# redwarp/kmeans-gpu

Hardware: AMD Instinct MI355X
Metric: pixels/sec per Lloyd iteration (8192x8192, k=256) (higher is better)
Workload: dtype f32; 1 GPU; synthetic uniform RGBA 8192x8192 (seed 0x5EED0003), k=256, one Lloyd iteration = update + assign (labels written every iteration) + accumulate; width=8192, height=8192, k=256, collective_backend=none (one rank), collective_ranks=1, label_pass=before the next iteration, update=by the last launch of the assign pass (kmg_lloyd_assign_update)

## Files before the change

### kmeans-gpu_amd/csrc/kmg_cube.hip

```cpp

#include "kmg_internal.h"
#include "kmg_table_dev.h"

#include <hip/hip_fp16.h>
#include <stdlib.h>

namespace kmg {

typedef float f32x2 __attribute__((ext_vector_type(2)));


namespace {

constexpr uint32_t kMaxListed = 32;
constexpr uint32_t kMaxLong = 256;
constexpr uint32_t kLongFlag = 0x200u;

__device__ __forceinline__ uint32_t sel3(uint32_t i, uint32_t x0, uint32_t x1, uint32_t x2)
{
    return i == 0u ? x0 : (i == 1u ? x1 : x2);
}

__device__ __forceinline__ int round_dir(int g, int m)
{
// ... 8 lines not shown
{
    v |= dpp_u32<kDppXor1>(v);
    v |= dpp_u32<kDppXor2>(v);
    v |= dpp_u32<kDppHalfMirror>(v);
    return v;
}

__device__ __forceinline__ uint32_t group8_min_u32(uint32_t v)
{
    v = min(v, dpp_u32<kDppXor1>(v));
    v = min(v, dpp_u32<kDppXor2>(v));
    v = min(v, dpp_u32<kDppHalfMirror>(v));
    return v;
}

__device__ __forceinline__ uint32_t group8_max_u32(uint32_t v)
{
    v = max(v, dpp_u32<kDppXor1>(v));
    v = max(v, dpp_u32<kDppXor2>(v));
    v = max(v, dpp_u32<kDppHalfMirror>(v));
    return v;
}



__device__ __forceinline__ uint32_t cell_pair_entry(const uint32_t idx[8], uint32_t occ, uint32_t lane)
{
    uint32_t rem = occ;
    uint32_t lab0 = 0, lab1 = 0, lab2 = 0, cnt0 = 0, cnt1 = 0, cnt2 = 0, msk0 = 0, msk1 = 0, msk2 = 0, n_occ = 0;
#pragma unroll
    for (int t = 0; t < 3; ++t) {
        const unsigned long long any = __ballot(rem != 0u);
        if (any) {
            uint32_t mine = 0;
#pragma unroll
            for (int q = 7; q >= 0; --q) mine = ((rem >> q) & 1u) ? idx[q] : mine;
            const uint32_t v = lane_value(mine, (uint32_t)__builtin_ctzll(any));
            uint32_t mm = 0;
#pragma unroll
            for (int q = 0; q < 8; ++q) mm |= (idx[q] == v ? 1u : 0u) << q;
            mm &= rem;
            rem &= ~mm;
            const uint32_t packed = wave_add_u32((uint32_t)__builtin_popcount(mm) | (t == 0 ? (uint32_t)__builtin_popcount(occ) << 10 : 0u));
            const uint32_t c = packed & 1023u;
            if (t == 0) { lab0 = v; msk0 = mm; cnt0 = c; n_occ = packed >> 10; }
            if (t == 1) { lab1 = v; msk1 = mm; cnt1 = c; }
            if (t == 2) { lab2 = v; msk2 = mm; cnt2 = c; }
// ... 17 lines not shown
    const int gx = (int)((hR & 1023u) * nA) - (int)((hA & 1023u) * nR);
    const int gy = (int)(((hR >> 10) & 1023u) * nA) - (int)(((hA >> 10) & 1023u) * nR);
    const int gz = (int)((hR >> 20) * nA) - (int)((hA >> 20) * nR);
    const int ax = gx < 0 ? -gx : gx, ay = gy < 0 ? -gy : gy, az = gz < 0 ? -gz : gz;
    const int m = ax > ay ? (ax > az ? ax : az) : (ay > az ? ay : az);
    int nx = 2, ny = 0, nz = 0;
    if (m > 0) { nx = round_dir(gx, m); ny = round_dir(gy, m); nz = round_dir(gz, m); }

    const int xl = (int)(((lane >> 5) & 1u) * 4u + ((lane >> 1) & 3u));
    const int yl = (int)(((lane >> 4) & 1u) * 4u + (lane & 1u) * 2u);
    const int zl = (int)(((lane >> 3) & 1u) * 4u);
    const int bias = 7 * ((nx < 0 ? -nx : 0) + (ny < 0 ? -ny : 0) + (nz < 0 ? -nz : 0));
    const int p0 = nx * xl + ny * yl + nz * zl + bias;
    int p[8];
#pragma unroll
    for (int q = 0; q < 8; ++q) p[q] = p0 + ny * (q >> 2) + nz * (q & 3);
    const uint32_t notB = occ & ~mB;
    uint32_t tl = 63u, hi = 64u;
#pragma unroll
    for (int q = 0; q < 8; ++q) {
        if ((rest >> q) & 1u) tl = min(tl, (uint32_t)p[q]);
        if ((notB >> q) & 1u) hi = min(hi, (uint32_t)(63 - p[q]));
    }
    u16x2 packed = __builtin_bit_cast(u16x2, tl | (hi << 16));
    packed = __builtin_elementwise_min(packed, __builtin_bit_cast(u16x2, dpp_u32<kDppXor1>(__builtin_bit_cast(uint32_t, packed))));
    packed = __builtin_elementwise_min(packed, __builtin_bit_cast(u16x2, dpp_u32<kDppXor2>(__builtin_bit_cast(uint32_t, packed))));
    packed = __builtin_elementwise_min(packed, __builtin_bit_cast(u16x2, dpp_u32<kDppHalfMirror>(__builtin_bit_cast(uint32_t, packed))));
    packed = __builtin_elementwise_min(packed, __builtin_bit_cast(u16x2, dpp_u32<kDppMirror>(__builtin_bit_cast(uint32_t, packed))));
    packed = __builtin_elementwise_min(packed, __builtin_bit_cast(u16x2, (uint32_t)__builtin_amdgcn_update_dpp(-1, (int)__builtin_bit_cast(uint32_t, packed), 0x142, 0xA, 0xF, false)));
    packed = __builtin_elementwise_min(packed, __builtin_bit_cast(u16x2, (uint32_t)__builtin_amdgcn_update_dpp(-1, (int)__builtin_bit_cast(uint32_t, packed), 0x143, 0xC, 0xF, false)));
    const uint32_t pk = lane_value(__builtin_bit_cast(uint32_t, packed), 63);
    const int tlo = (int)(pk & 0xFFFFu);
    const int thi = 63 - (int)(pk >> 16);
    const int w = thi + 1 > tlo ? thi + 1 - tlo : 0;
    const uint32_t code = pair_dir_code(nx, ny, nz);
    if (w <= 6) return pair_entry(labA, labB, code, (uint32_t)tlo, (uint32_t)w);
    uint32_t low = 0, high = 0;
#pragma unroll
    for (int q = 0; q < 8; ++q) {
        if ((occ >> q) & 1u) { low += p[q] < tlo ? 1u : 0u; high += p[q] > thi ? 1u : 0u; }
    }
    const uint32_t lh = wave_add_u32(low | (high << 10));
    if ((lh & 1023u) >= (lh >> 10)) return pair_entry(labA, labB, code, (uint32_t)tlo, 7u);
    const int range = 7 * ((nx < 0 ? -nx : nx) + (ny < 0 ? -ny : ny) + (nz < 0 ? -nz : nz));
    return pair_entry(labB, labA, pair_dir_code(-nx, -ny, -nz), (uint32_t)(range - thi), 7u);
}

__device__ __forceinline__ uint32_t merge_state(uint32_t a, uint32_t b)
{
    return (a == kSubEmpty) ? b : ((b == kSubEmpty || b == a) ? a : (uint32_t)kSubMixed);
}

template <typename LabelT>
__device__ __forceinline__ void store_labels64(LabelT *dst64, uint32_t label, uint32_t lane)
{
    if (sizeof(LabelT) == 1) {
        const uint32_t t = label | (dpp_u32<kDppXor1>(label) << 8);
        const uint32_t u = t | (dpp_u32<kDppXor2>(t) << 16);
        if ((lane & 3u) == 0u) reinterpret_cast<uint32_t *>(dst64)[lane >> 2] = u;
    } else {
        const uint32_t t = label | (dpp_u32<kDppXor1>(label) << 16);
        if ((lane & 1u) == 0u) reinterpret_cast<uint32_t *>(dst64)[lane >> 1] = t;
    }
}


struct alignas(16) CellWork {
    uint16_t list[kMaxListed];
    unsigned long long br[4];
    uint32_t npop;
    uint32_t scan_set;
    uint32_t pad[6];
};
static_assert(sizeof(CellWork) == 128, "CellWork layout");

constexpr uint32_t kPairPending = 0xFFFFFFFEu;

constexpr uint32_t kLongSegs = 16, kLongSegCap = kCells / kLongSegs, kLongCount = 0, kLongCells = 64;
constexpr size_t kListsWords = kLongCells + kCells;
constexpr uint32_t kItemCands = 12;

__device__ __forceinline__ void flush_bins(const unsigned long long *bins, uint32_t k, uint32_t repl, uint32_t bin_stride,
                                           int64_t *sums, uint32_t n_rows)
{
    __syncthreads();
    unsigned long long *row = reinterpret_cast<unsigned long long *>(sums) + (uint64_t)(blockIdx.x % n_rows) * 4ull * k;
    for (uint32_t i = threadIdx.x; i < 4u * k; i += blockDim.x) {
        unsigned long long v = 0ull;
        for (uint32_t r = 0; r < repl; ++r) v += bins[(uint64_t)r * bin_stride + i];
        if (v) atomicAdd(row + i, v);
    }
}

__device__ __forceinline__ uint2 long_list_stage(const float4 *s_cent, const unsigned long long *s_masks, uint16_t *s_long,
                                              unsigned long long *s_sub, float4 sb0, float4 sb1, float4 sb2, uint32_t npop,
                                              uint32_t words, uint64_t *sub_masks_cell)
{
    const uint32_t lane = threadIdx.x & 63u;
    const uint32_t sub_of_lane = lane >> 3, cand_of_lane = lane & 7u;
// ... 1263 lines not shown
        KMG_STAMP(0);
        uint32_t task = wv < waves_used ? blockIdx.x * waves_used + wv : tasks;
        if (bal_state) task = min(s_bal[64u + wv], tasks);
        const uint32_t prime = tasks % 2053u ? 2053u : 1031u;
        const uint32_t pos = (uint32_t)(((uint64_t)task * prime) % tasks) + ci * tasks;
        const bool valid = task < tasks && ci < cpw && pos < n_work;
        const uint32_t cell = valid ? ((SUMS && n_work != kCells) ? work[1u + pos] : pos) : 0u;
        const uint32_t sc = cell * 8u + sub;
        const uint32_t cell_a = (uint32_t)__builtin_amdgcn_ds_bpermute((int)(((lane >> 4) * 8u) << 2), (int)cell);
        const uint32_t cell_b = (uint32_t)__builtin_amdgcn_ds_bpermute((int)(((4u + (lane >> 4)) * 8u) << 2), (int)cell);
        const float cbv_a = reinterpret_cast<const float *>(bounds + cell_a)[lane & 15u];
        const float cbv_b = reinterpret_cast<const float *>(bounds + cell_b)[lane & 15u];
        const float4 *sbp = reinterpret_cast<const float4 *>(sub_bounds + sc);
        const float4 sb0 = sbp[0], sb1 = sbp[1], sb2 = sbp[2];
        longlong2 g01 = {0, 0}, g23 = {0, 1};
        long long cell_sum = 0;
        if (SUMS) {
            const longlong2 *sp = reinterpret_cast<const longlong2 *>(sub_agg + (uint64_t)sc * 4u);
            g01 = sp[0]; g23 = sp[1];
            cell_sum = agg[4ull * cell + (sub & 3u)];
        }
        uint2 occ8 = make_uint2(0xFFFFFFFFu, 0xFFFFFFFFu);
        if (occ_bits) occ8 = *reinterpret_cast<const uint2 *>(occ_bits + (uint64_t)cell * 64u + sub * 8u);
        if (sub == 0u) s_cell[slot] = cell;

        float *s_cb = reinterpret_cast<float *>(s_lbl + (size_t)wv * 8u * kCellColours);
        s_cb[lane] = cbv_a;
        s_cb[64u + lane] = cbv_b;
        __builtin_amdgcn_wave_barrier();
        for (uint32_t c = 0; c < cpw; ++c) {
            const uint32_t ccell = lane_value(cell, c * 8u);
            const bool cvalid = lane_value((uint32_t)valid, c * 8u) != 0u;
            const float4 *cq = reinterpret_cast<const float4 *>(s_cb + c * 16u);
            const float4 q0 = cq[0], q1 = cq[1], q2 = cq[2];
            CellBounds cb;
            cb.L0 = q0.x; cb.L1 = q0.y; cb.a0 = q0.z; cb.a1 = q0.w;
            cb.b0 = q1.x; cb.b1 = q1.y; cb.C0 = q1.z; cb.C1 = q1.w;
            cb.wC0 = q2.x; cb.wC1 = q2.y; cb.wH0 = q2.z; cb.wH1 = q2.w;
            float lo[4], U = 3.0e38f;
#pragma unroll
            for (int w = 0; w < 4; ++w) {
                const KeyRange r = key_range(cb, c4[w].x, c4[w].y, c4[w].z, c4[w].w);
                lo[w] = r.lo;
                U = fminf(U, r.hi);
            }
            const float Us = mask_threshold(wave_min(U));
// ... 31 lines not shown
        if (listed) {
            CellBounds sb;
            sb.L0 = sb0.x; sb.L1 = sb0.y; sb.a0 = sb0.z; sb.a1 = sb0.w;
            sb.b0 = sb1.x; sb.b1 = sb1.y; sb.C0 = sb1.z; sb.C1 = sb1.w;
            sb.wC0 = sb2.x; sb.wC1 = sb2.y; sb.wH0 = sb2.z; sb.wH1 = sb2.w;
            uint32_t Ubest = 0x7F7FFFE0u;
            for (uint32_t p = 0; p < npop; ++p) {
                const float4 c = s_cent[s_list[slot * kMaxListed + p]];
                Ubest = min(Ubest, ((float_to_bits(key_range(sb, c.x, c.y, c.z, c.w).hi) + 31u) & ~31u) | p);
            }
            const float Us = mask_threshold(bits_to_float(Ubest & ~31u));
            for (uint32_t p = 0; p < npop; ++p) {
                const float4 c = s_cent[s_list[slot * kMaxListed + p]];
                sm |= (key_range(sb, c.x, c.y, c.z, c.w).lo <= Us ? 1u : 0u) << p;
            }
            istar = Ubest & 31u;
            ubits = Ubest & ~31u;
        }
        const uint32_t np0 = (uint32_t)__builtin_popcount(sm);
        const bool was_decided = listed && occupied && np0 == 1u;
        const bool mine = listed && occupied && np0 > 1u;
        s_mask[threadIdx.x] = sm;
        *reinterpret_cast<uint2 *>(s_occ + slot * 64u + sub * 8u) = occ8;
        const uint32_t others = (mine && dominance) ? sm & ~(1u << istar) : 0u;
        if (others) {
            s_ref[threadIdx.x] = ubits | istar;
            const uint32_t nt = (uint32_t)__builtin_popcount(others);
            uint32_t at = atomicAdd(&s_count[8u + wv], nt);
            for (uint32_t m = others; m && at < kOneTests; m &= m - 1u, ++at)
                s_test[wv * kOneTests + at] = (uint16_t)((lane << 5) | (uint32_t)__builtin_ctz(m));
        }
        KMG_STAMP(2);
        __builtin_amdgcn_fence(__ATOMIC_RELEASE, "workgroup");
        __builtin_amdgcn_wave_barrier();
        __builtin_amdgcn_fence(__ATOMIC_ACQUIRE, "workgroup");
        if (dominance) {
            const uint32_t n_tests = min(__builtin_amdgcn_readfirstlane(s_count[8u + wv]), kOneTests);
            for (uint32_t t = lane; t < n_tests; t += 64u) {
                const uint32_t ent = (uint32_t)s_test[wv * kOneTests + t];
                const uint32_t e = wv * 64u + (ent >> 5), tp = ent & 31u;
                const uint32_t r = s_ref[e];
                const float4 cj = s_cent[s_list[(e >> 3) * kMaxListed + tp]], ci4 = s_cent[s_list[(e >> 3) * kMaxListed + (r & 31u)]];
                HalfModel mdl;
                mdl.load(sub_affine, (uint64_t)s_cell[e >> 3] * 8u + (e & 7u));
                if (dominated(mdl, cj, ci4, bits_to_float(r & ~31u))) atomicAnd(&s_mask[e], ~(1u << tp));
            }
// ... 66 lines not shown
                    for (uint32_t m = un; m; m &= m - 1u, ++q) {
                        const uint32_t cc = (uint32_t)s_list[slot * kMaxListed + (uint32_t)__builtin_ctz(m)] << (8u * (q & 3u));
                        iw0 |= q < 4u ? cc : 0u; iw1 |= (q >= 4u && q < 8u) ? cc : 0u; iw2 |= q >= 8u ? cc : 0u;
                    }
                }
                s_item[i_base + bits_below_lane(item_b)] = make_uint4(slot | (sub << 7) | (s1 << 10) | (n_un << 14) | (type << 30), iw0, iw1, iw2);
            }
            if (stats) {
                st_single += (uint32_t)__builtin_popcountll(__ballot(single && sub == 0u));
                st_multi += (uint32_t)__builtin_popcountll(__ballot(valid && !single && sub == 0u));
                st_unlisted += (uint32_t)__builtin_popcountll(__ballot(unlisted && sub == 0u));
                st_decided += (uint32_t)__builtin_popcountll(__ballot(was_decided));
                st_scanned += (uint32_t)__builtin_popcountll(__ballot(mine || (unlisted && occupied)));
                st_cands += wave_add_u32(mine ? np0 : ((unlisted && occupied) ? npop : 0u));
                st_removed += wave_add_u32((uint32_t)__builtin_popcount(sm & ~nm));
                st_one += (uint32_t)__builtin_popcountll(__ballot(one));
            }
        }
        KMG_STAMP(4);
        __syncthreads();
        const uint32_t n_items = s_count[0];
        KMG_STAMP_VALUE(8, n_items); KMG_STAMP_VALUE(10, s_count[8]);

        auto cell_entry = [&](const uint32_t ps) {
            const uint32_t pcell = __builtin_amdgcn_readfirstlane(s_cell[ps]);
            const uint2 lv = *reinterpret_cast<const uint2 *>(s_lbl + ps * kCellColours + lane * 8u);
            uint32_t e = kPairPending;
            if (!(flags & kCubeNoEntries)) {
                const uint32_t occ = (uint32_t)s_occ[ps * 64u + lane];
                uint32_t idx[8];
#pragma unroll
                for (uint32_t q = 0; q < 4u; ++q) { idx[q] = (lv.x >> (8u * q)) & 0xFFu; idx[4u + q] = (lv.y >> (8u * q)) & 0xFFu; }
                e = cell_pair_entry(idx, occ, lane);
            }
            if (lane == 0u) pair_entries[pcell] = e;
            *reinterpret_cast<uint2 *>(colour_labels + (uint64_t)pcell * kCellColours + lane * 8u) = lv;
        };

        {
            uint32_t A_h = 0u, A_w0 = 0u, A_w1 = 0u, A_w2 = 0u, B_h = 0u, B_w0 = 0u, B_w1 = 0u, B_w2 = 0u, C_h = 0u, C_w0 = 0u, C_w1 = 0u, C_w2 = 0u;
            float4 A_v0, A_v1, B_v0, B_v1, C_v0, C_v1;
            uint32_t A_c0 = 1u, A_c1 = 1u, B_c0 = 1u, B_c1 = 1u, C_c0 = 1u, C_c1 = 1u;
            long long A_g = 0, B_g = 0, C_g = 0;
            bool A_ok = false, B_ok = false, C_ok = false;
#define KMG_REQUEST_ITEM(X)                                                                                       \
            do {                                                                                                  \
                uint32_t next_ = 0u;                                                                              \
                if (lane == 0u) next_ = atomicAdd(&s_count[4], 1u);                                               \
                next_ = __builtin_amdgcn_readfirstlane(next_);                                                    \
                X##_ok = next_ < n_items;                                                                         \
                const uint4 it_ = s_item[next_ < n_items ? next_ : 0u];                                           \
                X##_h = __builtin_amdgcn_readfirstlane(it_.x); X##_w0 = __builtin_amdgcn_readfirstlane(it_.y);    \
                X##_w1 = __builtin_amdgcn_readfirstlane(it_.z); X##_w2 = __builtin_amdgcn_readfirstlane(it_.w);   \
                const uint32_t cell_ = __builtin_amdgcn_readfirstlane(s_cell[X##_h & 127u]);                       \
                const uint32_t c0_ = cell_ * kCellColours + ((X##_h >> 7) & 7u) * 64u + lane;                     \
                const uint32_t c1_ = cell_ * kCellColours + ((X##_h >> 10) & 7u) * 64u + lane;    \
// ... 165 lines not shown
}
#define env_grid(name, dflt) grid_or(KMG_TOOLS_ENV(name), (dflt))

uint32_t cube_replicas(uint32_t k)
{
    uint32_t r = 4;
    if (const char *e = KMG_TOOLS_ENV("KMG_CUBE_REPL")) { const int v = atoi(e); if (v == 1 || v == 2 || v == 4 || v == 8) r = (uint32_t)v; }
    while (r > 1u && (uint64_t)r * (k * 32ull + 32ull) > 33024ull) r >>= 1;
    return r;
}

size_t cube_work_bytes() { return sizeof(CellWork) * (size_t)kCells + sizeof(uint32_t) * kListsWords; }

bool cube_single_launch(uint32_t k, uint32_t flags)
{
    return k <= kSmallMaxK || (k <= 256u && !(flags & kCubeHot));
}

hipError_t launch_cube(const CubePass &c, hipStream_t st)
{
    const uint32_t k = c.k;
    uint32_t n_rows = c.n_rows, flags = c.flags;
    const CubeBalance *balance = c.balance;
    const CubeTail tl = (c.tail && c.hist && n_rows <= 1u) ? *c.tail : CubeTail();
    const uint32_t kpad = (k + 63u) & ~63u;
    const bool with_sums = c.hist != nullptr;
    const uint32_t repl = with_sums ? cube_replicas(k) : 1u;
    const size_t lds_stage = sizeof(float4) * kpad + (with_sums ? sizeof(unsigned long long) * 4ull * k : 0) +
                             sizeof(uint32_t) * (kBlock / 64) * kMaxListed + sizeof(unsigned long long) * (kBlock / 64) * (kpad / 64u) +
                             (k <= 256 ? (kBlock / 64) * (32u * sizeof(unsigned long long) + kMaxLong * sizeof(uint16_t)) : 0u);
    const size_t lds_scan = sizeof(float4) * kpad + (with_sums ? sizeof(unsigned long long) * (4ull * k + 4ull) * repl : 0) +
                            sizeof(float4) * (kScanBlock / 64) * kMaxListed + (k <= 256 ? 1u : 2u) * (kScanBlock / 64) * kCellColours;
    {
        const size_t lds_max = device_info().lds_max;
        if (lds_stage > lds_max || lds_scan > lds_max) return hipErrorInvalidValue;
    }
    const size_t lds_max_dev = device_info().lds_max;
    static const bool small_on = tools_env_int(KMG_TOOLS_ENV("KMG_CUBE_SMALL"), 1) != 0;
    if (k <= kSmallMaxK && small_on) {
        static const uint32_t g_small = env_grid("KMG_SMALL_GRID", kCells / kSmallCells);
        const uint32_t kp = k <= 8u ? 8u : (k <= 16u ? 16u : 32u);
        const size_t lds = sizeof(float4) * kp + (with_sums ? sizeof(unsigned long long) * (4ull * k + 4ull) * kSmallRepl : 0) +
                           (size_t)kSmallCells * kCellColours + sizeof(uint32_t) * kSmallBlock * 2u + sizeof(uint32_t) * kSmallCells +
                           sizeof(uint32_t) * 4u + sizeof(uint16_t) * (kSmallBlock + kSmallCells + kSmallTests) + kSmallBlock;
        if (!n_rows) n_rows = 1u;
        static const bool split = tools_env_int(KMG_TOOLS_ENV("KMG_CUBE_SMALL"), 1) == 2;
// ... 88 lines not shown
```

### kmeans-gpu_amd/csrc/kmg_lloyd.hip

```cpp

#include <math.h>

#include "kmg_state.h"

static void drop_events(kmg_lloyd *s)
{
    for (ProfEvent &e : s->events) { s->pool.push_back(e.e0); s->pool.push_back(e.e1); }
    s->events.clear();
}

static void destroy_events(kmg_lloyd *s)
{
    drop_events(s);
    for (hipEvent_t e : s->pool) (void)hipEventDestroy(e);
    s->pool.clear();
}

static int side_flush(kmg_lloyd *s, hipStream_t st)
{
    for (int i = 0; i < 2; ++i)
        if (s->lab_pending[i]) {
            HIP_TRY(hipStreamWaitEvent(st, s->ev_lab[i], 0));
            s->lab_pending[i] = false;
        }
// ... 30 lines not shown
{
    if (t.balance_work != work) { t.balance_work = work; t.balance_pass = 0; }
    CubeBalance b;
    b.state = t.d_balance;
    b.pass = t.balance_pass++;
    return b;
}

static hipError_t cube_pass(kmg_lloyd *s, hipStream_t st, int64_t *d_sums, uint32_t rows, bool share, bool balance, uint32_t flags = 0u,
                            const CubeTail *tail = nullptr, unsigned long long *d_stage = nullptr)
{
    ColourTable &t = s->tab;
    const uint32_t *work = share ? share_or_work(t) : t.d_work;
    CubeBalance bal;
    if (balance) bal = next_balance(t, work);
    CubePass c;
    c.hist = t.d_hist; c.agg = t.d_agg; c.sub_agg = t.d_sub_agg; c.occ_bits = t.d_occ; c.work = work;
    c.bounds = s->p->d_bounds; c.sub_bounds = s->p->d_sub_bounds; c.lab_table = s->p->d_lab_table;
    c.cent = s->d_cent; c.k = s->k;
    c.masks = t.d_masks; c.cell_work = t.d_cell_work; c.colour_labels = t.d_colour_labels; c.sub_table = t.d_sub;
    c.sums = d_sums; c.n_rows = rows; c.flags = flags | hot_flag(t); c.stats = d_stage; c.tail = tail;
    c.sub_affine = affine_for(s->p, s->k, st);
    c.balance = balance ? &bal : nullptr;
    return launch_cube(c, st);
}

static int label_pass(kmg_lloyd *s, const uint8_t *d_rgba, uint64_t n, uint32_t *d_labels, hipStream_t st, const CubeTail *tail = nullptr,
                      int64_t *acc = nullptr)
{
    const ColourTable &t = s->tab;
    PROF_LAUNCH(s, KMG_K_LABELS, st, launch_labels((const uint32_t *)d_rgba, n, t.d_colour_labels, t.d_sub, s->k, nullptr, d_labels, st,
                                                   s->reserve_cus, hot_list(t), tail, acc));
    return KMG_OK;
}

static CubeTail make_tail(const kmg_lloyd *s, int64_t *acc_out, bool do_update)
{
    return CubeTail{acc_out, do_update ? 1 : 0, s->p->opt.convergence, s->d_cent, s->d_nconv};
}

static int check_unweighted(const kmg_lloyd *s, const char *call)
{
    if (s->weighted)
        return fail(KMG_ERR_INVALID_ARGUMENT, "%s: the object's sums are weighted (kmg_lloyd_set_weighting): the colour table counts pixels", call);
    return KMG_OK;
}

// ... 108 lines not shown
    if (e == hipSuccess) e = launch_sub_affine(p->d_lab_table, p->d_sub_bounds, a, st);
    if (e == hipSuccess) e = hipStreamSynchronize(st);
    if (e != hipSuccess) {
        (void)hipGetLastError();
        if (a) (void)hipFree(a);
        p->affine_failed = true;
        return nullptr;
    }
    p->d_sub_affine = a;
    return a;
}

static int tables_from_histogram(kmg_lloyd *s, uint64_t n_pixels, hipStream_t st)
{
    ColourTable &t = s->tab;
    HIP_TRY(launch_cell_aggregates(t.d_hist, s->p->d_lab_table, t.d_agg, t.d_sub_agg, t.d_occ, st));
    HIP_TRY(launch_work_list(t.d_agg, t.d_work, s->k <= 256 ? n_pixels : 0, st));
    HIP_TRY(hipMemcpyAsync(&t.n_hot, t.d_work + kCells + 1, sizeof(uint32_t), hipMemcpyDeviceToHost, st));
    HIP_TRY(hipMemcpyAsync(&t.n_occ, t.d_work, sizeof(uint32_t), hipMemcpyDeviceToHost, st));
    HIP_TRY(hipStreamSynchronize(st));
    if (const char *e = KMG_TOOLS_ENV("KMG_HOT_CELLS")) { if (e[0] == '0') t.n_hot = 0; }
    t.d_work_share = nullptr;
    t.balance_work = nullptr;
    return KMG_OK;
}

static int bind_image_impl(kmg_lloyd *s, const uint8_t *d_rgba, uint64_t n, void *stream, bool want_tie, uint64_t first_index)
{
    if (!s || !d_rgba || n == 0) return fail(KMG_ERR_INVALID_ARGUMENT, "bad bind_image arguments");
    if (s->side) HIP_TRY(hipStreamSynchronize(s->side));
    s->lab_pending[0] = s->lab_pending[1] = false;
    KMG_TRY(check_pixel_count(n));
    HIP_TRY(hipSetDevice(s->p->device));
    KMG_TRY(ensure_bounds(s->p, S(stream)));
    ColourTable &t = s->tab;
    if (!t.d_hist) {
        const size_t sizes[11] = {sizeof(uint32_t) << 24, sizeof(int64_t) * 4ull * kCells, sizeof(int64_t) * 4ull * kSubCells,
                                  (size_t)1 << 21, cube_work_bytes(), cube_masks_bytes(s->k),
                                  sizeof(uint32_t) * kWorkWords, (size_t)(s->k <= 256 ? 1 : 2) << 24, sub_table_bytes(),
                                  sizeof(uint32_t) * (kCells + 1), cube_balance_bytes()};
        size_t need = 0;
        for (size_t b : sizes) need += pad256(b);
        const hipError_t e = block_take(s->p, need, &t.blk, &t.blk_cap);
        if (e != hipSuccess) {
            t.blk = nullptr; t.blk_cap = 0;
            return fail_hip(e, "colour table allocation");
        }
        size_t off = 0;
        t.d_hist = (uint32_t *)carve(t.blk, off, sizes[0]);
        t.d_agg = (int64_t *)carve(t.blk, off, sizes[1]);
        t.d_sub_agg = (int64_t *)carve(t.blk, off, sizes[2]);
        t.d_occ = (uint8_t *)carve(t.blk, off, sizes[3]);
        t.d_cell_work = carve(t.blk, off, sizes[4]);
        t.d_masks = (uint64_t *)carve(t.blk, off, sizes[5]);
        t.d_work = (uint32_t *)carve(t.blk, off, sizes[6]);
        t.d_colour_labels = carve(t.blk, off, sizes[7]);
        t.d_sub = (uint16_t *)carve(t.blk, off, sizes[8]);
        t.share_buf = (uint32_t *)carve(t.blk, off, sizes[9]);
        t.d_balance = (uint16_t *)carve(t.blk, off, sizes[10]);
    }
    t.d_work_share = nullptr;
    t.balance_work = nullptr;
    t.rgba = nullptr;
    t.tables_valid = false;
    t.tie_valid = false;
    t.bound_by_init = false;
    t.bound_by_caller = false;
    HIP_TRY(hipMemsetAsync(t.d_sub, 0xFF, sub_table_bytes(), S(stream)));
    if (t.d_sub_alt) HIP_TRY(hipMemsetAsync(t.d_sub_alt, 0xFF, sub_table_bytes(), S(stream)));
    if (n >= (1ull << 21)) {
        StreamBuf small, elems, keys;
        hipError_t e = small.alloc(s->p, sizeof(uint32_t) * (4 * 1024 + 1), S(stream));
        if (e == hipSuccess) e = elems.alloc(s->p, sizeof(uint16_t) * n, S(stream));
        if (e == hipSuccess && want_tie) e = keys.alloc(s->p, sizeof(uint32_t) * n, S(stream));
        if (e == hipSuccess)
            e = launch_partitioned_histogram((const uint32_t *)d_rgba, n, first_index, (uint32_t *)small.ptr, (uint16_t *)elems.ptr,
                                             (uint32_t *)keys.ptr, t.d_hist, t.d_tie, S(stream));
        if (e != hipSuccess) return fail_hip(e, "histogram");
    } else {
        HIP_TRY(hipMemsetAsync(t.d_hist, 0, sizeof(uint32_t) << 24, S(stream)));
        HIP_TRY(launch_histogram((const uint32_t *)d_rgba, n, t.d_hist, S(stream)));
        if (want_tie) {
            HIP_TRY(hipMemsetAsync(t.d_tie, 0, sizeof(uint32_t) << 24, S(stream)));
            HIP_TRY(launch_tie_keys((const uint32_t *)d_rgba, n, first_index, t.d_tie, S(stream)));
        }
// ... 675 lines not shown
extern "C" int kmg_lloyd_labels(kmg_lloyd *s, const uint8_t *d_rgba, uint64_t n, uint32_t *d_labels, void *stream)
try {
    if (!s || !d_rgba || !d_labels || n == 0) return fail(KMG_ERR_INVALID_ARGUMENT, "bad labels arguments");
    HIP_TRY(hipSetDevice(s->p->device));
    KMG_TRY(side_flush(s, S(stream)));
    if (table_bound(s, d_rgba, n) && s->tab.tables_valid) {
        KMG_TRY(ensure_entries(s, S(stream)));
        return label_pass(s, d_rgba, n, d_labels, S(stream));
    }
    PROF_LAUNCH(s, KMG_K_ASSIGN, S(stream), launch_assign((const uint32_t *)d_rgba, n, s->d_cent, s->k, s->p->d_lut,
                                                          d_labels, nullptr, S(stream)));
    return KMG_OK;
}
KMG_ABI_CATCH

extern "C" int kmg_lloyd_set_cell_share(kmg_lloyd *s, uint32_t part, uint32_t parts, void *stream)
try {
    if (!s || parts == 0 || part >= parts) return fail(KMG_ERR_INVALID_ARGUMENT, "bad set_cell_share arguments");
    KMG_TRY(check_unweighted(s, "set_cell_share"));
    KMG_TRY(check_bound(s, "set_cell_share"));
    HIP_TRY(hipSetDevice(s->p->device));
    ColourTable &t = s->tab;
    t.balance_work = nullptr;
    if (parts == 1u) { t.d_work_share = nullptr; return KMG_OK; }
    HIP_TRY(launch_work_share(t.d_work, part, parts, t.share_buf, S(stream)));
    t.d_work_share = t.share_buf;
    return KMG_OK;
}
KMG_ABI_CATCH

extern "C" int kmg_lloyd_labels_from_tables(kmg_lloyd *s, const uint8_t *d_rgba, uint64_t n, uint32_t *d_labels, void *stream)
try {
    if (!s || !d_rgba || !d_labels || n == 0) return fail(KMG_ERR_INVALID_ARGUMENT, "bad labels_from_tables arguments");
    KMG_TRY(check_bound(s, "labels_from_tables"));
    HIP_TRY(hipSetDevice(s->p->device));
    KMG_TRY(side_flush(s, S(stream)));
    KMG_TRY(ensure_entries(s, S(stream)));
    return label_pass(s, d_rgba, n, d_labels, S(stream));
}
KMG_ABI_CATCH

extern "C" int kmg_lloyd_labels_from_tables_update(kmg_lloyd *s, const uint8_t *d_rgba, uint64_t n, uint32_t *d_labels, int64_t *d_acc4,
                                                   void *stream)
try {
    if (!s || !d_rgba || !d_labels || !d_acc4 || n == 0) return fail(KMG_ERR_INVALID_ARGUMENT, "bad labels_from_tables_update arguments");
    KMG_TRY(check_unweighted(s, "labels_from_tables_update"));
// ... 285 lines not shown
```

### kmeans-gpu_amd/csrc/kmg_state.h

```cpp
#pragma once

#include <hip/hip_runtime.h>

#include <stdarg.h>
#include <stdio.h>
#include <stdlib.h>
#include <string.h>

#include <algorithm>
#include <atomic>
#include <chrono>
#include <exception>
#include <memory>
#include <mutex>
#include <thread>
#include <new>
#include <vector>

#include "kmg_checks.h"
#include "kmg_color.h"
#include "kmg_internal.h"
#include "kmg_kernels.h"
#include "kmg_octree.h"
#include "kmg_table.h"
// ... 77 lines not shown

static inline uint32_t working_cutoff(uint32_t alpha_cutoff, int weighting) { return weighting && alpha_cutoff == 0 ? 1u : alpha_cutoff; }
constexpr uint64_t kMaxWeightedPixels = 1ull << 28;

static inline size_t pad256(size_t bytes) { return (bytes + 255u) & ~(size_t)255u; }

struct ProfEvent { int id; hipEvent_t e0, e1; };

struct ColourTable {
    const uint8_t *rgba = nullptr;
    uint64_t n = 0;
    uint32_t *d_hist = nullptr;
    int64_t *d_agg = nullptr;
    int64_t *d_sub_agg = nullptr;
    uint8_t *d_occ = nullptr;
    void *d_cell_work = nullptr;
    uint64_t *d_masks = nullptr;
    uint32_t *d_work = nullptr;
    uint32_t n_hot = 0;
    uint32_t n_occ = 0;
    uint16_t *d_balance = nullptr;
    const uint32_t *balance_work = nullptr;
    uint32_t balance_pass = 0;
    uint32_t *share_buf = nullptr;
    uint32_t *d_work_share = nullptr;
    bool tables_valid = false;
    bool entries_valid = false;
    void *d_colour_labels = nullptr;
    uint16_t *d_sub = nullptr;
    void *d_colour_labels_alt = nullptr;
    uint16_t *d_sub_alt = nullptr;
    uint32_t *d_tie = nullptr;
    float *d_cdist = nullptr;
    void *d_init_cells = nullptr;
    bool tie_valid = false;
    bool bound_by_init = false;
    bool bound_by_caller = false;
    uint64_t tie_first = 0;
    void *blk = nullptr, *blk_alt = nullptr, *blk_init = nullptr;
    size_t blk_cap = 0, blk_alt_cap = 0, blk_init_cap = 0;
};

struct kmg_lloyd {
    kmg_processor *p = nullptr;
    uint32_t k = 0;
    Centroid *d_cent = nullptr;
// ... 133 lines not shown
```

### kmeans-gpu_amd/csrc/kmg_table.h

```cpp
#pragma once

#include <hip/hip_runtime.h>
#include <stdint.h>

#include "kmg_kernels.h"

namespace kmg {

constexpr uint32_t kCells = 32768;
constexpr uint32_t kCellColours = 512;
constexpr uint32_t kSubCells = kCells * 8;
constexpr uint32_t kCubeGrid = 2048;
constexpr uint32_t kMergeRows = 64;
constexpr uint32_t kHotMax = 56;
constexpr uint32_t kWorkWords = kCells + 1 + 1 + kHotMax;

constexpr uint16_t kSubEmpty = 0xFFFF;
constexpr uint16_t kSubMixed = 0xFFFE;

struct alignas(16) CellBounds {
    float L0, L1, a0, a1, b0, b1, C0, C1, wC0, wC1, wH0, wH1;
    float pad[4];
};

// ... 40 lines not shown
    const int bias = 7 * ((nx < 0 ? -nx : 0) + (ny < 0 ? -ny : 0) + (nz < 0 ? -nz : 0));
    return ((uint32_t)nx & 255u) | (((uint32_t)ny & 255u) << 8) | (((uint32_t)nz & 255u) << 16) | ((uint32_t)bias << 24);
}

__host__ __device__ inline uint32_t pair_entry(uint32_t A, uint32_t B, uint32_t code, uint32_t tlo, uint32_t w)
{
    return (A & 255u) | ((B & 255u) << 8) | (code << 16) | (tlo << 23) | (w << 29);
}

__host__ __device__ inline int pair_project(uint32_t dir_word, uint32_t px)
{
    return (int)(int8_t)(dir_word & 255u) * (int)(px & 7u) + (int)(int8_t)((dir_word >> 8) & 255u) * (int)((px >> 8) & 7u) +
           (int)(int8_t)((dir_word >> 16) & 255u) * (int)((px >> 16) & 7u) + (int)(dir_word >> 24);
}

__host__ __device__ inline uint32_t pair_decode(uint32_t e, int p)
{
    const int tlo = (int)((e >> 23) & 63u);
    const int w = (int)(e >> 29);
    const int thr = tlo + w + (w == 7 ? 64 : 0);
    if (p < tlo) return e & 255u;
    if (p >= thr) return (e >> 8) & 255u;
    return kPairFine;
}

hipError_t launch_cell_bounds(const float *lut, CellBounds *bounds, CellBounds *sub_bounds, float4 *lab_table, hipStream_t st);
hipError_t launch_histogram(const uint32_t *rgba, uint64_t n, uint32_t *hist, hipStream_t st);
hipError_t launch_partitioned_histogram(const uint32_t *rgba, uint64_t n, uint64_t first_index, uint32_t *small,
                                        uint16_t *elems, uint32_t *keys, uint32_t *hist, uint32_t *tie, hipStream_t st);
hipError_t launch_cell_aggregates(const uint32_t *hist, const float4 *lab_table, int64_t *agg, int64_t *sub_agg, uint8_t *occ_bits,
                                  hipStream_t st);
hipError_t launch_work_list(const int64_t *agg, uint32_t *work, uint64_t n_pixels, hipStream_t st);
hipError_t launch_sparsity_probe(const uint32_t *rgba, uint64_t n, uint32_t *out3, hipStream_t st);
hipError_t launch_work_share(const uint32_t *work, uint32_t part, uint32_t parts, uint32_t *out, hipStream_t st);
hipError_t launch_tie_keys(const uint32_t *rgba, uint64_t n, uint64_t first_index, uint32_t *tie, hipStream_t st);
size_t init_scratch_bytes();
hipError_t launch_init_records(const uint32_t *work, const CellBounds *bounds, void *init_scratch, hipStream_t st);
hipError_t launch_init_pass_cells(const uint32_t *tie, const uint8_t *occ_bits, const float4 *lab_table, Centroid *cent,
                                  uint32_t j, int do_pass, float *dist, void *init_scratch, unsigned long long *band_key,
                                  const uint32_t *pick_rgba, const float *lut, hipStream_t st);
hipError_t launch_init_cells_multi(const uint32_t *tie, const uint8_t *occ_bits, const float4 *lab_table, Centroid *cent, uint32_t k,
                                   uint32_t launch, float *dist, void *init_scratch, const uint32_t *pick_rgba, const float *lut,
                                   hipStream_t st);
const uint32_t *init_cells_multi_count(const void *init_scratch, uint32_t launch);
size_t cube_work_bytes();
constexpr uint32_t kCubeNoEntries = 0x10000u;
constexpr uint32_t kCubeHot = 0x40000u;
constexpr uint32_t kCubeSplitLong = 0x80000u;
constexpr uint32_t kCubeSmallMaxK = 32;
bool cube_single_launch(uint32_t k, uint32_t flags);
hipError_t launch_cube_entries(const uint32_t *work, const uint8_t *occ_bits, const void *colour_labels, uint16_t *sub_table,
                               uint32_t k, hipStream_t st);
struct CubeTail {
    int64_t *acc_out = nullptr;
    int do_update = 0;
    float convergence = 0.0f;
    Centroid *cent = nullptr;
    uint32_t *n_converged = nullptr;
};
struct CubeBalance {
    uint16_t *state = nullptr;
    uint32_t pass = 0;
};
size_t cube_balance_bytes();
struct CubePass {
    const uint32_t *hist = nullptr;
    const int64_t *agg = nullptr;
    const int64_t *sub_agg = nullptr;
    const uint8_t *occ_bits = nullptr;
    const uint32_t *work = nullptr;
    const CellBounds *bounds = nullptr;
    const CellBounds *sub_bounds = nullptr;
    const Centroid *cent = nullptr;
    uint32_t k = 0;
    const float4 *lab_table = nullptr;
    uint64_t *masks = nullptr;
    void *cell_work = nullptr;
    void *colour_labels = nullptr;
    uint16_t *sub_table = nullptr;
    int64_t *sums = nullptr;
    uint32_t n_rows = 0;
    uint32_t flags = 0;
    unsigned long long *stats = nullptr;
    const CubeTail *tail = nullptr;
    const float *sub_affine = nullptr;
    const CubeBalance *balance = nullptr;
};
hipError_t launch_cube(const CubePass &pass, hipStream_t st);
size_t sub_affine_bytes();
hipError_t launch_sub_affine(const float4 *lab_table, const CellBounds *sub_bounds, float *affine, hipStream_t st);
hipError_t launch_labels(const uint32_t *rgba, uint64_t n, const void *colour_labels,
                         const uint16_t *sub_table, uint32_t k, const uint32_t *pal, uint32_t *labels,
                         hipStream_t st, uint32_t reserve_cus = 0, const uint32_t *hot = nullptr,
                         const CubeTail *tail = nullptr, int64_t *tail_sums = nullptr);

hipError_t launch_offset_candidates(const CellBounds *bounds, const Centroid *cent, uint32_t k, float threshold,
                                    uint64_t *masks, hipStream_t st);
hipError_t launch_dither_pruned(const uint32_t *rgba, uint32_t w, uint32_t rows, uint32_t row0, const Centroid *cent,
                                uint32_t k, const float *lut, const uint32_t *pal, float threshold,
                                const uint64_t *masks, uint32_t *out, hipStream_t st);

constexpr uint32_t kListBytes = 32, kListMax = 2 * kListBytes - 1;
constexpr uint32_t kLabCells = 40u * 72u * 72u;
constexpr size_t kLabListBytes = 2ull * kLabCells * kListBytes;
constexpr uint32_t kLabListMaxK = 512;
size_t lab_list_bytes(uint32_t k);
hipError_t launch_lab_candidates(const Centroid *cent, uint32_t k, float threshold, bool two_closest, uint8_t *lists, hipStream_t st);
hipError_t launch_meld_lists(const uint32_t *rgba, uint64_t n, const Centroid *cent, uint32_t k, const float *lut,
                             const uint8_t *lists, uint32_t *out, hipStream_t st);
// ... 20 lines not shown
```

Measured before the change: 307.9 billion pixels/s.

## Reuse previous iteration's pair entry as a hint to skip full pair search

Each cell's pair entry from the previous Lloyd pass is read back and, when still valid, used to rebuild the entry with a single projection and one wave reduction instead of the full multi-round label grouping and direction search in cell_pair_entry. Every eighth cell per pass (rotating) ignores the hint so entries are refreshed periodically. The hint is only used when the work list and sub-table are unchanged, and it can be disabled by environment variable. The cost is an extra global load per cell and some state tracking on the host, and entries may be less tight than a fresh search.

Result: no change. 309.3 billion pixels/s, median of 6 (+0.5%).

```diff
diff --git a/kmeans-gpu_amd/csrc/kmg_cube.hip b/kmeans-gpu_amd/csrc/kmg_cube.hip
--- a/kmeans-gpu_amd/csrc/kmg_cube.hip
+++ b/kmeans-gpu_amd/csrc/kmg_cube.hip
@@ -54,7 +54,17 @@
     return v;
 }
 
-
+__device__ __forceinline__ uint32_t wave_min_u16x2(uint32_t v)
+{
+    u16x2 packed = __builtin_bit_cast(u16x2, v);
+    packed = __builtin_elementwise_min(packed, __builtin_bit_cast(u16x2, dpp_u32<kDppXor1>(__builtin_bit_cast(uint32_t, packed))));
+    packed = __builtin_elementwise_min(packed, __builtin_bit_cast(u16x2, dpp_u32<kDppXor2>(__builtin_bit_cast(uint32_t, packed))));
+    packed = __builtin_elementwise_min(packed, __builtin_bit_cast(u16x2, dpp_u32<kDppHalfMirror>(__builtin_bit_cast(uint32_t, packed))));
+    packed = __builtin_elementwise_min(packed, __builtin_bit_cast(u16x2, dpp_u32<kDppMirror>(__builtin_bit_cast(uint32_t, packed))));
+    packed = __builtin_elementwise_min(packed, __builtin_bit_cast(u16x2, (uint32_t)__builtin_amdgcn_update_dpp(-1, (int)__builtin_bit_cast(uint32_t, packed), 0x142, 0xA, 0xF, false)));
+    packed = __builtin_elementwise_min(packed, __builtin_bit_cast(u16x2, (uint32_t)__builtin_amdgcn_update_dpp(-1, (int)__builtin_bit_cast(uint32_t, packed), 0x143, 0xC, 0xF, false)));
+    return lane_value(__builtin_bit_cast(uint32_t, packed), 63);
+}
 
 __device__ __forceinline__ uint32_t cell_pair_entry(const uint32_t idx[8], uint32_t occ, uint32_t lane)
 {
@@ -118,14 +128,7 @@
         if ((rest >> q) & 1u) tl = min(tl, (uint32_t)p[q]);
         if ((notB >> q) & 1u) hi = min(hi, (uint32_t)(63 - p[q]));
     }
-    u16x2 packed = __builtin_bit_cast(u16x2, tl | (hi << 16));
-    packed = __builtin_elementwise_min(packed, __builtin_bit_cast(u16x2, dpp_u32<kDppXor1>(__builtin_bit_cast(uint32_t, packed))));
-    packed = __builtin_elementwise_min(packed, __builtin_bit_cast(u16x2, dpp_u32<kDppXor2>(__builtin_bit_cast(uint32_t, packed))));
-    packed = __builtin_elementwise_min(packed, __builtin_bit_cast(u16x2, dpp_u32<kDppHalfMirror>(__builtin_bit_cast(uint32_t, packed))));
-    packed = __builtin_elementwise_min(packed, __builtin_bit_cast(u16x2, dpp_u32<kDppMirror>(__builtin_bit_cast(uint32_t, packed))));
-    packed = __builtin_elementwise_min(packed, __builtin_bit_cast(u16x2, (uint32_t)__builtin_amdgcn_update_dpp(-1, (int)__builtin_bit_cast(uint32_t, packed), 0x142, 0xA, 0xF, false)));
-    packed = __builtin_elementwise_min(packed, __builtin_bit_cast(u16x2, (uint32_t)__builtin_amdgcn_update_dpp(-1, (int)__builtin_bit_cast(uint32_t, packed), 0x143, 0xC, 0xF, false)));
-    const uint32_t pk = lane_value(__builtin_bit_cast(uint32_t, packed), 63);
+    const uint32_t pk = wave_min_u16x2(tl | (hi << 16));
     const int tlo = (int)(pk & 0xFFFFu);
     const int thi = 63 - (int)(pk >> 16);
     const int w = thi + 1 > tlo ? thi + 1 - tlo : 0;
@@ -140,6 +143,39 @@
     if ((lh & 1023u) >= (lh >> 10)) return pair_entry(labA, labB, code, (uint32_t)tlo, 7u);
     const int range = 7 * ((nx < 0 ? -nx : nx) + (ny < 0 ? -ny : ny) + (nz < 0 ? -nz : nz));
     return pair_entry(labB, labA, pair_dir_code(-nx, -ny, -nz), (uint32_t)(range - thi), 7u);
+}
+
+__device__ __forceinline__ bool cell_pair_entry_hinted(const uint32_t idx[8], uint32_t occ, uint32_t lane, uint32_t hint, uint32_t cell,
+                                                       uint32_t pass, uint32_t &entry)
+{
+    if (!pair_hint_usable(hint, cell, pass)) return false;
+    const uint32_t labA = hint & 255u, labB = (hint >> 8) & 255u, code = (hint >> 16) & 127u;
+    uint32_t mA = 0, mB = 0;
+#pragma unroll
+    for (int q = 0; q < 8; ++q) { mA |= (idx[q] == labA ? 1u : 0u) << q; mB |= (idx[q] == labB ? 1u : 0u) << q; }
+    const uint32_t rest = occ & ~mA, notB = occ & ~mB;
+    if (!__ballot((occ & mA) != 0u)) return false;
+    if (!__ballot(rest != 0u)) { entry = pair_entry(labA, labA, 0u, 0u, 0u); return true; }
+    const int nx = (int)(code / 25u) - 2, ny = (int)((code / 5u) % 5u) - 2, nz = (int)(code % 5u) - 2;
+    const int xl = (int)(((lane >> 5) & 1u) * 4u + ((lane >> 1) & 3u));
+    const int yl = (int)(((lane >> 4) & 1u) * 4u + (lane & 1u) * 2u);
+    const int zl = (int)(((lane >> 3) & 1u) * 4u);
+    const int bias = 7 * ((nx < 0 ? -nx : 0) + (ny < 0 ? -ny : 0) + (nz < 0 ? -nz : 0));
+    const int p0 = nx * xl + ny * yl + nz * zl + bias;
+    uint32_t tl = 63u, hi = 64u;
+#pragma unroll
+    for (int q = 0; q < 8; ++q) {
+        const int p = p0 + ny * (q >> 2) + nz * (q & 3);
+        if ((rest >> q) & 1u) tl = min(tl, (uint32_t)p);
+        if ((notB >> q) & 1u) hi = min(hi, (uint32_t)(63 - p));
+    }
+    const uint32_t pk = wave_min_u16x2(tl | (hi << 16));
+    const int tlo = (int)(pk & 0xFFFFu);
+    const int thi = 63 - (int)(pk >> 16);
+    const int w = thi + 1 > tlo ? thi + 1 - tlo : 0;
+    if (w > 6 || w > (int)(hint >> 29)) return false;
+    entry = pair_entry(labA, labB, code, (uint32_t)tlo, (uint32_t)w);
+    return true;
 }
 
 __device__ __forceinline__ uint32_t merge_state(uint32_t a, uint32_t b)
@@ -171,6 +207,10 @@
 static_assert(sizeof(CellWork) == 128, "CellWork layout");
 
 constexpr uint32_t kPairPending = 0xFFFFFFFEu;
+static_assert((kPairRefresh & (kPairRefresh - 1u)) == 0u && kPairRefresh <= 8u, "the pass number travels in flags bits 20..22");
+constexpr uint32_t kCubeHintPassShift = 20;
+__host__ __device__ inline uint32_t cube_hint_pass_flags(uint32_t pass) { return (pass % kPairRefresh) << kCubeHintPassShift; }
+__device__ __forceinline__ uint32_t cube_hint_pass(uint32_t flags) { return (flags >> kCubeHintPassShift) & (kPairRefresh - 1u); }
 
 constexpr uint32_t kLongSegs = 16, kLongSegCap = kCells / kLongSegs, kLongCount = 0, kLongCells = 64;
 constexpr size_t kListsWords = kLongCells + kCells;
@@ -1480,6 +1520,8 @@
         }
         uint2 occ8 = make_uint2(0xFFFFFFFFu, 0xFFFFFFFFu);
         if (occ_bits) occ8 = *reinterpret_cast<const uint2 *>(occ_bits + (uint64_t)cell * 64u + sub * 8u);
+        uint32_t hint = kPairFine;
+        if (flags & kCubePairHint) hint = pair_entries[cell];
         if (sub == 0u) s_cell[slot] = cell;
 
         float *s_cb = reinterpret_cast<float *>(s_lbl + (size_t)wv * 8u * kCellColours);
@@ -1557,6 +1599,7 @@
         const bool mine = listed && occupied && np0 > 1u;
         s_mask[threadIdx.x] = sm;
         *reinterpret_cast<uint2 *>(s_occ + slot * 64u + sub * 8u) = occ8;
+        if (sub == 0u) s_npop[slot] = hint;
         const uint32_t others = (mine && dominance) ? sm & ~(1u << istar) : 0u;
         if (others) {
             s_ref[threadIdx.x] = ubits | istar;
@@ -1669,7 +1712,7 @@
         const uint32_t n_items = s_count[0];
         KMG_STAMP_VALUE(8, n_items); KMG_STAMP_VALUE(10, s_count[8]);
 
-        auto cell_entry = [&](const uint32_t ps) {
+        auto cell_entry = [&](const uint32_t ps) __attribute__((always_inline)) {
             const uint32_t pcell = __builtin_amdgcn_readfirstlane(s_cell[ps]);
             const uint2 lv = *reinterpret_cast<const uint2 *>(s_lbl + ps * kCellColours + lane * 8u);
             uint32_t e = kPairPending;
@@ -1678,7 +1721,8 @@
                 uint32_t idx[8];
 #pragma unroll
                 for (uint32_t q = 0; q < 4u; ++q) { idx[q] = (lv.x >> (8u * q)) & 0xFFu; idx[4u + q] = (lv.y >> (8u * q)) & 0xFFu; }
-                e = cell_pair_entry(idx, occ, lane);
+                const uint32_t hint_e = __builtin_amdgcn_readfirstlane(s_npop[ps]);
+                if (!cell_pair_entry_hinted(idx, occ, lane, hint_e, pcell, cube_hint_pass(flags), e)) e = cell_pair_entry(idx, occ, lane);
             }
             if (lane == 0u) pair_entries[pcell] = e;
             *reinterpret_cast<uint2 *>(colour_labels + (uint64_t)pcell * kCellColours + lane * 8u) = lv;
@@ -1890,6 +1934,8 @@
     const uint32_t k = c.k;
     uint32_t n_rows = c.n_rows, flags = c.flags;
     const CubeBalance *balance = c.balance;
+    if (c.pair_hints && k > kSmallMaxK && cube_single_launch(k, flags) && tools_env_int(KMG_TOOLS_ENV("KMG_PAIR_HINT"), 1) != 0)
+        flags |= kCubePairHint | cube_hint_pass_flags(c.hint_pass);
     const CubeTail tl = (c.tail && c.hist && n_rows <= 1u) ? *c.tail : CubeTail();
     const uint32_t kpad = (k + 63u) & ~63u;
     const bool with_sums = c.hist != nullptr;
diff --git a/kmeans-gpu_amd/csrc/kmg_lloyd.hip b/kmeans-gpu_amd/csrc/kmg_lloyd.hip
--- a/kmeans-gpu_amd/csrc/kmg_lloyd.hip
+++ b/kmeans-gpu_amd/csrc/kmg_lloyd.hip
@@ -76,7 +76,12 @@
     c.sums = d_sums; c.n_rows = rows; c.flags = flags | hot_flag(t); c.stats = d_stage; c.tail = tail;
     c.sub_affine = affine_for(s->p, s->k, st);
     c.balance = balance ? &bal : nullptr;
-    return launch_cube(c, st);
+    c.pair_hints = t.hint_work == work && t.hint_sub == t.d_sub;
+    if (!c.pair_hints) { t.hint_work = work; t.hint_sub = t.d_sub; t.hint_pass = 0; }
+    c.hint_pass = t.hint_pass++;
+    const hipError_t e = launch_cube(c, st);
+    if (e != hipSuccess) t.hint_work = nullptr;
+    return e;
 }
 
 static int label_pass(kmg_lloyd *s, const uint8_t *d_rgba, uint64_t n, uint32_t *d_labels, hipStream_t st, const CubeTail *tail = nullptr,
@@ -231,6 +236,7 @@
     if (const char *e = KMG_TOOLS_ENV("KMG_HOT_CELLS")) { if (e[0] == '0') t.n_hot = 0; }
     t.d_work_share = nullptr;
     t.balance_work = nullptr;
+    t.hint_work = nullptr;
     return KMG_OK;
 }
 
@@ -270,6 +276,7 @@
     }
     t.d_work_share = nullptr;
     t.balance_work = nullptr;
+    t.hint_work = nullptr;
     t.rgba = nullptr;
     t.tables_valid = false;
     t.tie_valid = false;
@@ -991,6 +998,7 @@
     HIP_TRY(hipSetDevice(s->p->device));
     ColourTable &t = s->tab;
     t.balance_work = nullptr;
+    t.hint_work = nullptr;
     if (parts == 1u) { t.d_work_share = nullptr; return KMG_OK; }
     HIP_TRY(launch_work_share(t.d_work, part, parts, t.share_buf, S(stream)));
     t.d_work_share = t.share_buf;
diff --git a/kmeans-gpu_amd/csrc/kmg_state.h b/kmeans-gpu_amd/csrc/kmg_state.h
--- a/kmeans-gpu_amd/csrc/kmg_state.h
+++ b/kmeans-gpu_amd/csrc/kmg_state.h
@@ -123,6 +123,9 @@
     uint16_t *d_balance = nullptr;
     const uint32_t *balance_work = nullptr;
     uint32_t balance_pass = 0;
+    const uint32_t *hint_work = nullptr;
+    const uint16_t *hint_sub = nullptr;
+    uint32_t hint_pass = 0;
     uint32_t *share_buf = nullptr;
     uint32_t *d_work_share = nullptr;
     bool tables_valid = false;
diff --git a/kmeans-gpu_amd/csrc/kmg_table.h b/kmeans-gpu_amd/csrc/kmg_table.h
--- a/kmeans-gpu_amd/csrc/kmg_table.h
+++ b/kmeans-gpu_amd/csrc/kmg_table.h
@@ -86,6 +86,38 @@
     if (p < tlo) return e & 255u;
     if (p >= thr) return (e >> 8) & 255u;
     return kPairFine;
+}
+
+constexpr uint32_t kPairRefresh = 8;
+
+__host__ __device__ inline bool pair_hint_usable(uint32_t hint, uint32_t cell, uint32_t pass)
+{
+    return ((hint >> 16) & 127u) < kPairDirs && (hint & 255u) != ((hint >> 8) & 255u) && (hint >> 29) != 7u &&
+           (cell + pass) % kPairRefresh != 0u;
+}
+
+__host__ __device__ inline bool pair_entry_hinted_reference(const uint8_t *labels, const uint8_t *occ, uint32_t hint, uint32_t cell,
+                                                            uint32_t pass, uint32_t *entry)
+{
+    if (!pair_hint_usable(hint, cell, pass)) return false;
+    const uint32_t A = hint & 255u, B = (hint >> 8) & 255u, code = (hint >> 16) & 127u;
+    const uint32_t dir = pair_dir_word(code);
+    bool any_a = false, any_rest = false;
+    int tlo = 63, thi = -1;
+    for (uint32_t c = 0; c < kCellColours; ++c) {
+        if (!((occ[c >> 3] >> (c & 7u)) & 1u)) continue;
+        uint32_t r, g, b;
+        index_to_rgb(c, r, g, b);
+        const int p = pair_project(dir, r | (g << 8) | (b << 16));
+        if (labels[c] == A) any_a = true; else { any_rest = true; if (p < tlo) tlo = p; }
+        if (labels[c] != B && p > thi) thi = p;
+    }
+    if (!any_a) return false;
+    if (!any_rest) { *entry = pair_entry(A, A, 0u, 0u, 0u); return true; }
+    const int w = thi + 1 > tlo ? thi + 1 - tlo : 0;
+    if (w > 6 || w > (int)(hint >> 29)) return false;
+    *entry = pair_entry(A, B, code, (uint32_t)tlo, (uint32_t)w);
+    return true;
 }
 
 hipError_t launch_cell_bounds(const float *lut, CellBounds *bounds, CellBounds *sub_bounds, float4 *lab_table, hipStream_t st);
@@ -110,6 +142,7 @@
 size_t cube_work_bytes();
 constexpr uint32_t kCubeNoEntries = 0x10000u;
 constexpr uint32_t kCubeHot = 0x40000u;
+constexpr uint32_t kCubePairHint = 0x20000u;
 constexpr uint32_t kCubeSplitLong = 0x80000u;
 constexpr uint32_t kCubeSmallMaxK = 32;
 bool cube_single_launch(uint32_t k, uint32_t flags);
@@ -149,6 +182,8 @@
     const CubeTail *tail = nullptr;
     const float *sub_affine = nullptr;
     const CubeBalance *balance = nullptr;
+    bool pair_hints = false;
+    uint32_t hint_pass = 0;
 };
 hipError_t launch_cube(const CubePass &pass, hipStream_t st);
 size_t sub_affine_bytes();
```
